# kekoveca/MPI-and-Open-MP

Hardware: AMD Instinct MI355X
Metric: Gcell-updates/sec at 1/2/4/8 MI355X + % of HBM roofline, bit-exact (higher is better)
Workload: dtype u32 (1 bit/cell)

## Files before the change

### include/life_mi355x.h

```cpp
#ifndef LIFE_MI355X_H
#define LIFE_MI355X_H

#include <stdint.h>

#ifdef __cplusplus
extern "C" {
#endif

#define LIFE_OK 0
#define LIFE_EINVAL (-1)
#define LIFE_EHIP (-2)
#define LIFE_ERCCL (-3)
#define LIFE_ENOMEM (-4)
#define LIFE_ESTATE (-5)
#define LIFE_EIO (-6)

#define LIFE_KERNEL_BYTE 0
#define LIFE_KERNEL_BIT 1

#define LIFE_XPORT_AUTO 0
#define LIFE_XPORT_RCCL 1
#define LIFE_XPORT_LOCAL 2

typedef struct life_dev life_dev;
// ... 81 lines not shown
int life_dev_checksum(life_dev *d, uint64_t *sum);


int life_dev_clear(life_dev *d);

int life_dev_set_cells(life_dev *d, const int64_t *xy, int64_t n, int alive);

int life_dev_upload_bits(life_dev *d, const uint8_t *packed);

int life_dev_gather_rect(life_dev *d, int64_t x0, int64_t y0, int64_t w, int64_t h, uint8_t *cells);

int life_dev_set_rect(life_dev *d, int64_t x0, int64_t y0, int64_t w, int64_t h, const uint8_t *cells);

int life_dev_gather_density(life_dev *d, int64_t fx, int64_t fy, uint32_t *counts);

int life_dev_sync(life_dev *d);
int life_dev_barrier(life_dev *d);
int life_device_count(void);
int life_dev_layout(life_dev *d, int local_shard, life_layout *out);
int life_dev_world(life_dev *d, int *world, int *dims0, int *dims1, int *nlocal, int *transport);
int life_dev_shard_info(life_dev *d, int local_shard, int *device, char pci_bus_id[64], int *rccl_nranks);

int life_dev_set_timing(life_dev *d, int on);

#define LIFE_OPT_SMALL_GRID 1
#define LIFE_OPT_OVERLAP 2
#define LIFE_OPT_BLOCK_GENS 5
#define LIFE_OPT_SMALL_WINDOW 4
#define LIFE_OPT_LOOPBACK 6
#define LIFE_OPT_FLOW 7
#define LIFE_OPT_FLOW_CHUNK 8
#define LIFE_OPT_DEEP_HALO 9
#define LIFE_OPT_PIPELINE 11
int life_dev_configure(life_dev *d, int option, int value);
#define LIFE_PATH_NONE 0
#define LIFE_PATH_ONEGEN 1
#define LIFE_PATH_TILES 2
#define LIFE_PATH_FLOW 3
#define LIFE_PATH_SMALL 5
int life_dev_last_path(life_dev *d);
int life_dev_kernel_stats(life_dev *d, double *avg_ms, int64_t *launches, double *bytes_per_launch);
int life_dev_kernel_work(life_dev *d, double *cell_updates_per_launch, double *valu_ops_per_launch);
int life_dev_phase_stats(life_dev *d, double *ring_ms, double *interior_ms, double *halo_ms, double *block_ms,
                         int64_t *blocks);
int life_dev_call_stats(life_dev *d, double *host_enqueue_ms, double *pass_enqueue_max_ms, int64_t *passes,
                        double *device_span_ms);

int life_tune(int kernel, int rows, int depth);

int life_tune_temporal(int kernel, int rows);

int life_measure_copy(int device, int64_t bytes, int reps, double *gbps);

void life_dev_destroy(life_dev *d);

#ifdef __cplusplus
}
#endif
#endif
```

### mpi-and-open-mp_amd/csrc/life_dev.hip

```cpp
#include <stdarg.h>

#include <chrono>
#include <thread>

#include "life_dev_internal.h"
#include "life_env.h"

using namespace life::rt;

thread_local std::string life::rt::g_err;

void life::rt::set_err(const char *fmt, ...) {
    char buf[512];
    va_list ap;
    va_start(ap, fmt);
    vsnprintf(buf, sizeof buf, fmt, ap);
    va_end(ap);
    g_err = buf;
}

static const int kEnvBlockGens = life::env::read(life::env::kBlockGens);
static const int kEnvFlow = life::env::read(life::env::kFlow);
static const bool kEnvDeepHalo = life::env::read(life::env::kDeepHalo) != 0;
static const int kEnvPipeline = [] {
    const int v = life::env::read(life::env::kPipeline);
    return v == 2 ? life::env::kPipeline.dflt : v;
}();
static int default_block_gens(int kernel) {
    return kEnvBlockGens ? kEnvBlockGens : (kernel == LIFE_KERNEL_BIT ? 12 : 32);
}

namespace {

int alloc_fill_byte() { return life::env::read(life::env::kPoison) ? 0xA5 : 0; }

int shard_alloc(Shard &s) {
    HIPCHK(hipSetDevice(s.device));
    HIPCHK(hipStreamCreateWithPriority(&s.stream, hipStreamNonBlocking, 0));
    HIPCHK(hipStreamCreateWithPriority(&s.stream2, hipStreamNonBlocking, 0));
    HIPCHK(hipStreamCreateWithPriority(&s.comm_stream, hipStreamNonBlocking, 0));
    const int fill = alloc_fill_byte();
    const int64_t slack = s.lay.generations_per_exchange > 1 ? life::kTemporalSlackRows : 0;
    const size_t bytes = (size_t)(s.lay.pitch * (s.lay.rows + slack));
    for (int i = 0; i < 2; i++) {
        HIPCHK(hipMalloc(&s.buf[i], bytes));
        HIPCHK(hipMemsetAsync(s.buf[i], fill, bytes, s.stream));
    }
    HIPCHK(hipEventCreateWithFlags(&s.ev_int, hipEventDisableTiming));
    HIPCHK(hipEventCreateWithFlags(&s.ev_halo, hipEventDisableTiming));
    HIPCHK(hipEventCreateWithFlags(&s.ev_sync, hipEventDisableTiming));
    HIPCHK(hipEventCreateWithFlags(&s.ev_entry, hipEventDisableTiming));
    for (hipEvent_t &e : s.ev_pipe) HIPCHK(hipEventCreateWithFlags(&e, hipEventDisableTiming));
    const size_t col_bytes = (size_t)life::column_stage_bytes(s.lay);
    HIPCHK(hipMalloc(&s.col_send, col_bytes));
    HIPCHK(hipMalloc(&s.col_recv, col_bytes));
    HIPCHK(hipMalloc(&s.d_count, 2 * sizeof(unsigned long long)));
    HIPCHK(hipMalloc(&s.sink, 1024));
    HIPCHK(hipMemsetAsync(s.col_send, fill, col_bytes, s.stream));
    HIPCHK(hipMemsetAsync(s.col_recv, fill, col_bytes, s.stream));
    HIPCHK(hipMemsetAsync(s.d_count, 0, 2 * sizeof(unsigned long long), s.stream));
// ... 37 lines not shown
        if (!s.comm) continue;
        HIPCHK(hipSetDevice(s.device));
        int64_t *h = reinterpret_cast<int64_t *>(s.h_count);
        h[0] = value;
        h[1] = -(int64_t)value;
        HIPCHK(hipMemcpyAsync(s.d_count, h, 2 * sizeof(int64_t), hipMemcpyHostToDevice, s.stream));
        NCCLCHK(ncclAllReduce(s.d_count, s.d_count, 2, ncclInt64, ncclMax, s.comm, s.stream));
        HIPCHK(hipMemcpyAsync(h, s.d_count, 2 * sizeof(int64_t), hipMemcpyDeviceToHost, s.stream));
        CHK(bounded_sync(s, what, -1));
        const int64_t hi = h[0], lo = -h[1];
        if (hi != lo) {
            set_err("%s is collective in rank mode: ranks passed %lld .. %lld", what, (long long)lo, (long long)hi);
            return LIFE_EINVAL;
        }
    }
    return LIFE_OK;
}

life_dev *new_dev(int64_t nx, int64_t ny, int dims0, int dims1, int world, int kernel) {
    int dims[2] = {dims0, dims1};
    if (dims0 <= 0 || dims1 <= 0) life_dims_create(world, dims);
    if (dims[0] * dims[1] != world) return nullptr;
    life_dev *d = new life_dev;
    d->nx = nx;
    d->ny = ny;
    d->dims[0] = dims[0];
    d->dims[1] = dims[1];
    d->world = world;
    d->kernel = kernel;
    d->block_gens = default_block_gens(kernel);
    d->deep = kEnvDeepHalo;
    d->flow = kEnvFlow;
    d->pipe = kEnvPipeline;
    return d;
}

int create_shards(life_dev *d, const std::vector<int> &ranks, const std::vector<int> &devices) {
    for (size_t i = 0; i < ranks.size(); i++) {
        d->shards.emplace_back();
        Shard &s = d->shards.back();
        s.rank = ranks[i];
        s.device = devices[i];
        const int rc = life_layout_query(d->nx, d->ny, d->dims[0], d->dims[1], s.rank, d->kernel, &s.lay);
        if (rc != LIFE_OK) {
            set_err("layout: nx=%lld ny=%lld dims=%dx%d rank %d kernel %d", (long long)d->nx,
                    (long long)d->ny, d->dims[0], d->dims[1], s.rank, d->kernel);
            return rc;
        }
    }
    for (Shard &s : d->shards) CHK(shard_alloc(s));
    return plan_halos(d);
}

void tail_prewarm(const life_dev *d) {
    for (size_t i = 0; i < d->shards.size(); ++i) {
        bool seen = false;
        for (size_t j = 0; j < i; ++j)
            seen |= d->shards[j].lay.w == d->shards[i].lay.w && d->shards[j].lay.h == d->shards[i].lay.h;
        if (!seen) life::prewarm_tail_plans(d->shards[i].lay, max_pass_gens(d), part(d, 1));
    }
}

int finish_create(life_dev *d, int rc, life_dev **out) {
    if (rc != LIFE_OK) {
        life_dev_destroy(d);
        return rc;
// ... 236 lines not shown
        if (value < 0 || value > 4) return LIFE_EINVAL;
        d->small_mode = value;
        return LIFE_OK;
    case LIFE_OPT_SMALL_WINDOW: {
        const int R = value >> 8, K = value & 255;
        if (value != 0 && (K < 1 || R < 1 || R > 8 || R == 7)) return LIFE_EINVAL;
        if (value != 0 && life::reg_win_plan(d->shards[0].lay, R, K).blocks == 0) {
            set_err("small-grid window R=%d K=%d does not fit this grid", R, K);
            return LIFE_EINVAL;
        }
        d->win_rows = R;
        d->win_halo = K;
        return LIFE_OK;
    }
    case LIFE_OPT_OVERLAP: d->overlap = value != 0; return LIFE_OK;
    case LIFE_OPT_BLOCK_GENS:
        if (value < 0 || value > 32) return LIFE_EINVAL;
        d->block_gens = value > 0 ? value : default_block_gens(d->kernel);
        tail_prewarm(d);
        return LIFE_OK;
    case LIFE_OPT_FLOW:
        if (value < 0 || value > 3) return LIFE_EINVAL;
        d->flow = value;
        return LIFE_OK;
    case LIFE_OPT_DEEP_HALO:
        if (value < 0 || value > 1) return LIFE_EINVAL;
        if (d->rank_mode && d->world > 1) CHK(agree_all_ranks(d, value, "LIFE_OPT_DEEP_HALO"));
        d->deep = value != 0;
        return LIFE_OK;
    case LIFE_OPT_PIPELINE:
        if (value < 0 || value == 2 || value > life::kPipeMaxRegions) return LIFE_EINVAL;
        d->pipe = value;
        return LIFE_OK;
    case LIFE_OPT_FLOW_CHUNK:
        if (value < 0) return LIFE_EINVAL;
        d->flow_chunk = value;
        return LIFE_OK;
    case LIFE_OPT_LOOPBACK: {
        if (value < 0 || value > 3) return LIFE_EINVAL;
        if (d->world != 1 || d->shards.size() != 1) {
            set_err("loopback needs a single-shard world (world %d, %zu local shards)", d->world, d->shards.size());
            return LIFE_EINVAL;
        }
        Shard &s = d->shards[0];
        if (value && (s.lay.h < s.lay.yapron || s.lay.w < s.lay.xapron)) {
            set_err("loopback: %lld x %lld cells < the %lld-column / %lld-row halo", (long long)s.lay.w,
                    (long long)s.lay.h, (long long)s.lay.xapron, (long long)s.lay.yapron);
            return LIFE_EINVAL;
        }
        if (value && d->transport == LIFE_XPORT_RCCL && !s.comm) {
            set_err("loopback over RCCL needs a communicator (life_dev_create_rank with a unique id, or "
                    "life_dev_create_ex with LIFE_XPORT_RCCL)");
            return LIFE_EINVAL;
        }
        d->loop = value == 0 ? 0 : value == 1 ? 3 : value == 2 ? 1 : 2;
        CHK(plan_halos(d));
        CHK(exchange(d, 0, false));
        tail_prewarm(d);
        return life_dev_sync(d);
    }
    default: return LIFE_EINVAL;
    }
}

int life_tune(int kernel, int rows, int depth) {
    if ((rows && rows != 16 && rows != 32 && rows != 64) ||
// ... 20 lines not shown
```

### mpi-and-open-mp_amd/csrc/life_dev_internal.h

```cpp
#pragma once
#include <rccl/rccl.h>
#include <stdio.h>
#include <string.h>

#include <algorithm>
#include <string>
#include <vector>

#include "life_host.h"
#include "life_io.h"
#include "life_kernels.h"
#include "life_mi355x.h"

#pragma GCC visibility push(hidden)

namespace life {
namespace rt {

extern thread_local std::string g_err;
void set_err(const char *fmt, ...);

#define HIPCHK(expr)                                                                          \
    do {                                                                                      \
        hipError_t e_ = (expr);                                                               \
// ... 63 lines not shown
    std::vector<int> slot;
    std::vector<LocalCopy> copies;
    std::vector<int> waits[2][2];
    std::vector<TimedLaunch> timers;
    size_t timers_used = 0;
    std::vector<PhaseEvents> phases;
    size_t phases_used = 0;
};

}
}

struct life_dev {
    int64_t nx = 0, ny = 0;
    int dims[2] = {1, 1};
    int world = 1;
    int kernel = LIFE_KERNEL_BYTE;
    int transport = LIFE_XPORT_LOCAL;
    bool rank_mode = false;
    bool timing = false;
    bool phase_events = true;
    bool launch_events = true;
    bool overlap = true;
    int block_gens = 0;
    int small_mode = 1;
    int win_rows = 0, win_halo = 0;
    int loop = 0;
    int last_path = LIFE_PATH_NONE;
    bool deep = true;
    int since = 0;
    int flow = 0;
    int64_t flow_chunk = 0;
    int pipe = 0;
    struct {
        int R = 0, m = 0;
        int64_t pass = 0;
        life::PipePlan plan;
    } pipe_call;
    life::rt::TimedLaunch *call_timer = nullptr;
    std::vector<life::rt::Shard> shards;
    double acc_ms = 0.0;
    int64_t acc_launches = 0;
    double acc_bytes = 0.0;
    double acc_updates = 0.0;
    double acc_valu = 0.0;
    double ph_ring = 0.0, ph_int = 0.0, ph_halo = 0.0, ph_block = 0.0;
    int64_t ph_blocks = 0;
    double call_host_ms = 0.0, call_pass_max_ms = 0.0;
    int64_t call_passes = 0;
    bool call_spans = false;
};

namespace life {
namespace rt {

inline bool part(const life_dev *d, int a) { return d->dims[a] > 1 || ((d->loop >> a) & 1); }
inline bool self_wrap_x(const life_dev *d) { return !(d->loop & 1) && life::self_wrap_x(d->shards[0].lay, d->dims[0]); }
inline life::Wrap wrap_of(const life_dev *d) { return life::Wrap{!part(d, 0) && !self_wrap_x(d), !part(d, 1)}; }
inline bool temporal(const life_dev *d) { return d->shards[0].lay.generations_per_exchange > 1; }
inline bool deep_halo(const life_dev *d) {
    return d->deep && d->kernel == LIFE_KERNEL_BIT && temporal(d) && (part(d, 0) || part(d, 1)) && !self_wrap_x(d);
}
inline int max_pass_gens(const life_dev *d) {
    return std::min(std::min(d->shards[0].lay.generations_per_exchange, 32), d->block_gens);
}
inline Shard *find_local(life_dev *d, int rank) {
// ... 32 lines not shown
```

### mpi-and-open-mp_amd/csrc/life_env.h

```cpp
#pragma once
#include <limits.h>
#include <stdlib.h>

#include "life_mi355x.h"

namespace life {
namespace env {

struct IntKnob { const char *name; int dflt, lo, hi; };
struct FlagKnob { const char *name; int dflt; };
struct RealKnob { const char *name; double dflt, lo, hi; };

inline int read(const IntKnob &k, int dflt) {
    const char *e = getenv(k.name);
    const int v = e ? atoi(e) : dflt;
    return v >= k.lo && v <= k.hi ? v : dflt;
}
inline int read(const IntKnob &k) { return read(k, k.dflt); }
inline int read(const FlagKnob &k) {
    const char *e = getenv(k.name);
    return e ? (atoi(e) != 0 ? 1 : 0) : k.dflt;
}
inline double read(const RealKnob &k) {
    const char *e = getenv(k.name);
    const double v = e ? atof(e) : k.dflt;
    return v > k.lo && v <= k.hi ? v : k.dflt;
}

constexpr IntKnob kStepRows{"LIFE_STEP_ROWS", 16, INT_MIN, INT_MAX};
constexpr IntKnob kStepDepth{"LIFE_STEP_DEPTH", 8, INT_MIN, INT_MAX};
constexpr FlagKnob kXcdOrderOnegen{"LIFE_XCD_ORDER_ONEGEN", -1};
constexpr IntKnob kTemporalRows{"LIFE_TEMPORAL_ROWS", 24, 16, 24};
constexpr IntKnob kTemporalRowsByte{"LIFE_TEMPORAL_ROWS_BYTE", 48, 32, 48};
constexpr FlagKnob kByteOneGhost{"LIFE_BYTE_ONE_GHOST", 1};
constexpr FlagKnob kBands{"LIFE_BANDS", 1};
constexpr FlagKnob kFlowBands{"LIFE_FLOW_BANDS", 1};
constexpr FlagKnob kXcdOrder{"LIFE_XCD_ORDER", 1};
constexpr FlagKnob kXcdOrderByte{"LIFE_XCD_ORDER_BYTE", 1};
constexpr IntKnob kTailSplit{"LIFE_TAIL_SPLIT", 2, 0, 2};
constexpr IntKnob kBlockGens{"LIFE_BLOCK_GENS", 0, 1, 32};
constexpr IntKnob kFlow{"LIFE_FLOW", 3, 0, 3};
constexpr FlagKnob kDeepHalo{"LIFE_DEEP_HALO", 1};
constexpr IntKnob kPipeline{"LIFE_PIPELINE", 1, 0, 16};
constexpr IntKnob kTimingMode{"LIFE_TIMING_MODE", 0, 0, 3};
constexpr FlagKnob kPoison{"LIFE_POISON", 0};
constexpr FlagKnob kInteriorTail{"LIFE_INTERIOR_TAIL", 0};
constexpr RealKnob kCommTimeoutS{"LIFE_COMM_TIMEOUT_S", 600.0, 0.0, 1e300};
constexpr IntKnob kTemporalDepth{"LIFE_TEMPORAL_DEPTH", LIFE_TEMPORAL_DEPTH, 1, 32};
constexpr IntKnob kTemporalDepthByte{"LIFE_TEMPORAL_DEPTH_BYTE", LIFE_TEMPORAL_DEPTH_BYTE, 1, 32};

}
}
```

### mpi-and-open-mp_amd/csrc/life_kernels.h

```cpp
#pragma once
#include <hip/hip_runtime.h>
#include <stdint.h>

#include "life_host.h"
#include "life_mi355x.h"

namespace life {

struct Region {
    int64_t u0, u1, r0, r1;
};

struct StepArgs {
    const uint8_t *in;
    uint8_t *out;
    uint8_t *sink;
    int64_t pitch, xoff, units, w, h, ya;
    int64_t u0, u1, r0, r1, nbx;
    int32_t wrapy;
    int32_t xcd;
};

struct Wrap {
    bool x, y;
// ... 8 lines not shown
StepTuning step_tuning(bool bit);
void set_step_tuning(int kernel, int rows, int depth);

constexpr int kMaxRegions = 4;
struct TileRegion {
    int64_t tx0, tx1, ty0, ty1;
};
struct TileGeom {
    int64_t lanes;
    int64_t cells;
    int64_t rows, ntx, nty;
    int gsh;
    int64_t bcol;
};
TileGeom tile_geom(const life_layout &L, int m);
int64_t region_items(const TileGeom &g, const TileRegion &r);
int tile_ghost(const life_layout &L, int m);
constexpr int64_t kTemporalSlackRows = 8 * 96;
bool flow_ok(const life_layout &L, int m);
int64_t flow_items_per_pass(const life_layout &L, int m, bool work_only = false);
int flow_slots(const life_layout &L);
int tile_slots(const life_layout &L);
hipError_t prewarm_tflow(const life_layout &L, int m, int flow, unsigned int *head, hipStream_t s);
hipError_t launch_tflow(const life_layout &L, const uint8_t *in, uint8_t *out, int m, int64_t passes,
                        unsigned int *head, unsigned int *done, Wrap wrap, int flow, hipStream_t s,
                        hipEvent_t ev0 = nullptr, hipEvent_t ev1 = nullptr);
struct Extend {
    int64_t y = 0;
    bool x = false;
};
hipError_t launch_tstep(const life_layout &L, const uint8_t *in, uint8_t *out, const TileRegion *r, int nreg,
                        int m, Wrap wrap, hipStream_t s,
                        double *valu_lane_ops = nullptr, hipEvent_t ev0 = nullptr, hipEvent_t ev1 = nullptr,
                        Extend ext = Extend{}, int64_t concurrent = 0);
void prewarm_tail_plans(const life_layout &L, int mmax, bool ext_y);
life_layout extended_layout(const life_layout &L, const Extend &ext);
int temporal_rows(bool bit);
int tile_waves(bool bit);
double tstep_valu_per_tile_lane(int m, bool byte);
void set_temporal_rows(int kernel, int nr);

constexpr int64_t kSmallMaxLds = 160 * 1024;
int64_t small_lds_bytes(const life_layout &L);
hipError_t launch_small(const life_layout &L, const uint8_t *in, uint8_t *out, int64_t gens, hipStream_t s);
int reg_small_rows(const life_layout &L);
hipError_t launch_reg_small(const life_layout &L, const uint8_t *in, uint8_t *out, int64_t gens,
                            hipStream_t s);
struct RegWinPlan {
    int R, K, ns, own, blocks;
};
RegWinPlan reg_win_plan(const life_layout &L, int R, int K);
hipError_t launch_reg_win(const life_layout &L, const RegWinPlan &p, const uint8_t *in, uint8_t *out, int gens,
                          hipStream_t s, bool nat_in, bool nat_out);

}
```

### mpi-and-open-mp_amd/csrc/life_kernels.hip

```cpp
#include "life_kernels.h"
#include "life_bitops.h"
#include "life_diag.h"
#include "life_env.h"

#include <hip/hip_ext.h>

#include <algorithm>
#include <stdint.h>

namespace life {
namespace {

constexpr int kBlock = 256;

__device__ __forceinline__ uint32_t from_left(uint32_t old, uint32_t v) {
    return (uint32_t)__builtin_amdgcn_update_dpp((int)old, (int)v, 0x138, 0xf, 0xf, false);
}
__device__ __forceinline__ uint32_t from_right(uint32_t old, uint32_t v) {
    return (uint32_t)__builtin_amdgcn_update_dpp((int)old, (int)v, 0x130, 0xf, 0xf, false);
}

struct ByteEnc {
    static constexpr int64_t kCellsPerUnit = 16;
    static constexpr uint32_t kCell0 = 0xFFu;
    static __device__ __forceinline__ int64_t dword_of(int64_t x) { return x >> 2; }
    static __device__ __forceinline__ uint32_t pos_in_dword(int64_t x) { return 8u * (uint32_t)(x & 3); }
    static __device__ __forceinline__ uint32_t top_shift(int64_t x) { return 24u - pos_in_dword(x); }
    struct H {
        uint32_t v[4];
    };
    static __device__ __forceinline__ H hsum(uint4 d, uint32_t l, uint32_t r) {
        H h;
        h.v[0] = d.x + __builtin_amdgcn_alignbyte(d.x, l, 3) + __builtin_amdgcn_alignbyte(d.y, d.x, 1);
        h.v[1] = d.y + __builtin_amdgcn_alignbyte(d.y, d.x, 3) + __builtin_amdgcn_alignbyte(d.z, d.y, 1);
        h.v[2] = d.z + __builtin_amdgcn_alignbyte(d.z, d.y, 3) + __builtin_amdgcn_alignbyte(d.w, d.z, 1);
        h.v[3] = d.w + __builtin_amdgcn_alignbyte(d.w, d.z, 3) + __builtin_amdgcn_alignbyte(r, d.w, 1);
        return h;
    }
    static __device__ __forceinline__ uint32_t rule1(uint32_t n9, uint32_t c) {
        const uint32_t m = (n9 - c) | c;
        const uint32_t t = m ^ 0x03030303u;
// ... 159 lines not shown
                const uint32_t m = E::kCell0 << E::pos_in_dword(q);
                c.pshift = E::pos_in_dword(q);
                c.pmask.x = comp == 0 ? m : 0u;
                c.pmask.y = comp == 1 ? m : 0u;
                c.pmask.z = comp == 2 ? m : 0u;
                c.pmask.w = comp == 3 ? m : 0u;
            }
        }
    }
    const bool st = u < a.u1;
    uint8_t *dst = st ? a.out + (ys + a.ya) * a.pitch + a.xoff + 16 * u : a.sink + 16 * lane;
    const int64_t spitch = st ? a.pitch : 0;
    const int64_t n = a.r1 - ys < R ? a.r1 - ys : R;
    if (n == R)
        strip_full<E, R, D, WRAPX>(c, ys, dst, spitch);
    else
        strip_tail<E, WRAPX>(c, ys, (int)n, dst, spitch);
}


constexpr int kStackWaves = 8;
struct TArgs {
    const uint8_t *in;
    uint8_t *out;
    int64_t pitch, xoff, W, h, ya;
    int64_t tx0[kMaxRegions], tx1[kMaxRegions], ty0[kMaxRegions], ty1[kMaxRegions], first[kMaxRegions + 1];
    int32_t nreg, m;
    int32_t gsh;
    int64_t bcol;
    int64_t tail_first, tail_y, tail_yend, tail_ntx, tail_tx0;
    int32_t tail_band;
    int64_t xcd_n;
    int32_t xext;
};

template <int NW>
using Xch = uint32_t[2][NW][4][64];
template <int NW>
using XchP = uint32_t[2][NW + 2][8][64];
template <int NW>
struct XchB {
    XchP<NW> s;
};

#ifndef LIFE_FLOW_BP_AHEAD
#define LIFE_FLOW_BP_AHEAD 1
#endif
#ifndef LIFE_FAST_WRAP
#define LIFE_FAST_WRAP 1
#endif

template <int R, bool WRAPX, bool WRAPY, int FLOW, int NW, bool BAND = false>
__device__ __forceinline__ void tile_body_bit(const TArgs &a, const uint8_t *in, uint8_t *out, int64_t tx,
                                              int64_t ty, XchB<NW> &xb, int gsh = 6, int nb = 1,
                                              int64_t ybase = 0, int64_t yend = -1) {
    XchP<NW> &xch = xb.s;
    static_assert(R >= 3, "window");
    const int K = a.m;
    const int T = NW * R - 2 * K;
    const int lane = threadIdx.x & 63;
    const int laddr = ((lane - 1) & 63) << 2, raddr = ((lane + 1) & 63) << 2;
    const int wi = __builtin_amdgcn_readfirstlane(threadIdx.x >> 6);
    const int gl = BAND ? lane >> gsh : 0;
    const int pin = BAND ? lane & ((1 << gsh) - 1) : lane;
    const int64_t j = tx * 62 + pin - 1;
    int64_t jl;
    if (WRAPX) {
        if (LIFE_FAST_WRAP && a.W >= 64) {
            jl = j < 0 ? j + a.W : (j >= a.W ? j - a.W : j);
        } else {
            jl = j % a.W;
            if (jl < 0) jl += a.W;
        }
    } else {
        jl = j > a.W ? a.W : j;
    }
    const uint32_t voff = (uint32_t)(a.xoff + 8 * jl);
    const int64_t y0 = ybase + ty * T - K + (int64_t)wi * R;
    const uint8_t *row0 = in + a.ya * a.pitch;
    uint32_t ve[R], vo[R];
    {
        int64_t y = y0 + (BAND ? (int64_t)(gl < nb ? gl : nb - 1) * T : 0);
        if (WRAPY) {
            if (LIFE_FAST_WRAP && a.h > 65 * (int64_t)(NW * R)) {
                y = y < 0 ? y + a.h : (y >= a.h ? y - a.h : y);
            } else {
                y %= a.h;
                if (y < 0) y += a.h;
            }
        }
        const uint8_t *p = row0 + y * a.pitch;
#pragma unroll
        for (int r = 0; r < R; ++r) {
            uint64_t q;
            if (FLOW)
                q = __hip_atomic_load(reinterpret_cast<uint64_t *>(const_cast<uint8_t *>(p) + voff),
                                      __ATOMIC_RELAXED, __HIP_MEMORY_SCOPE_AGENT);
            else
                q = *reinterpret_cast<const uint64_t *>(p + voff);
            ve[r] = (uint32_t)q;
            vo[r] = (uint32_t)(q >> 32);
            ++y;
            if (WRAPY && y == a.h) {
                y = 0;
                p = row0;
            } else {
                p += a.pitch;
            }
        }
    }
    auto hsum = [&](uint32_t e, uint32_t o, uint32_t &e0, uint32_t &e1, uint32_t &o0, uint32_t &o1) {
        BitEnc::pair_sums(e, o, bperm(laddr, o), bperm(raddr, e), e0, e1, o0, o1);
    };
    if (wi == 0 || wi == NW - 1)
        for (int q = 0; q < 16; ++q) xch[q >> 3][wi == 0 ? 0 : NW + 1][q & 7][lane] = 0u;
    for (int g = 0; g < a.m; ++g) {
        const int par = g & 1;
        uint32_t pe0, pe1, po0, po1, ce0, ce1, co0, co1;
        {
            uint32_t be0, be1, bo0, bo1;
            hsum(ve[R - 1], vo[R - 1], be0, be1, bo0, bo1);
            xch[par][wi + 1][4][lane] = be0;
            xch[par][wi + 1][5][lane] = be1;
            xch[par][wi + 1][6][lane] = bo0;
            xch[par][wi + 1][7][lane] = bo1;
        }
        hsum(ve[0], vo[0], pe0, pe1, po0, po1);
        xch[par][wi + 1][0][lane] = pe0;
        xch[par][wi + 1][1][lane] = pe1;
        xch[par][wi + 1][2][lane] = po0;
        xch[par][wi + 1][3][lane] = po1;
        __syncthreads();
        hsum(ve[1], vo[1], ce0, ce1, co0, co1);
        {
            const uint32_t ae0 = xch[par][wi][4][lane], ae1 = xch[par][wi][5][lane];
            const uint32_t ao0 = xch[par][wi][6][lane], ao1 = xch[par][wi][7][lane];
            ve[0] = BitEnc::rule1(ae0, ae1, pe0, pe1, ce0, ce1, ve[0]);
            vo[0] = BitEnc::rule1(ao0, ao1, po0, po1, co0, co1, vo[0]);
        }
        constexpr int BAH = FLOW ? LIFE_FLOW_BP_AHEAD : 0;
        uint32_t bl[BAH > 0 ? BAH : 1], br[BAH > 0 ? BAH : 1];
#pragma unroll
        for (int k = 0; k < BAH; ++k)
            if (2 + k < R - 1) {
                bl[k] = bperm(laddr, vo[2 + k]);
                br[k] = bperm(raddr, ve[2 + k]);
            }
#pragma unroll
        for (int r = 1; r < R - 1; ++r) {
// ... 5 lines not shown
                no1 = xch[par][wi + 1][7][lane];
            } else if (BAH > 0) {
                const uint32_t l = bl[0], rr = br[0];
#pragma unroll
                for (int k = 0; k + 1 < BAH; ++k) {
                    bl[k] = bl[k + 1];
                    br[k] = br[k + 1];
                }
                if (r + 1 + BAH < R - 1) {
                    bl[BAH - 1] = bperm(laddr, vo[r + 1 + BAH]);
                    br[BAH - 1] = bperm(raddr, ve[r + 1 + BAH]);
                }
                __builtin_amdgcn_sched_barrier(0);
                BitEnc::pair_sums(ve[r + 1], vo[r + 1], l, rr, ne0, ne1, no0, no1);
            } else {
                hsum(ve[r + 1], vo[r + 1], ne0, ne1, no0, no1);
            }
            ve[r] = BitEnc::rule1(pe0, pe1, ce0, ce1, ne0, ne1, ve[r]);
            vo[r] = BitEnc::rule1(po0, po1, co0, co1, no0, no1, vo[r]);
            pe0 = ce0;
            pe1 = ce1;
            po0 = co0;
            po1 = co1;
            ce0 = ne0;
            ce1 = ne1;
            co0 = no0;
            co1 = no1;
        }
        {
            const uint32_t de0 = xch[par][wi + 2][0][lane], de1 = xch[par][wi + 2][1][lane];
            const uint32_t do0 = xch[par][wi + 2][2][lane], do1 = xch[par][wi + 2][3][lane];
            ve[R - 1] = BitEnc::rule1(pe0, pe1, ce0, ce1, de0, de1, ve[R - 1]);
            vo[R - 1] = BitEnc::rule1(po0, po1, co0, co1, do0, do1, vo[R - 1]);
        }
    }
    const int r0 = min(max(K - wi * R, 0), R), r1 = min(max(NW * R - K - wi * R, 0), R);
    int lane2 = (int)(threadIdx.x & 63);
    asm volatile("" : "+v"(lane2));
    const int gl2 = BAND ? lane2 >> gsh : 0;
    const int pin2 = BAND ? lane2 & ((1 << gsh) - 1) : lane2;
    const int64_t j2 = tx * 62 + pin2 - 1;
    const bool st = (BAND ? (pin2 >= 1 && pin2 <= (1 << gsh) - 2 && j2 < a.W && gl2 < nb)
                          : (lane2 >= 1 && lane2 <= 62 && j2 < a.W)) ||
                    (!WRAPX && a.xext && (!BAND || gl2 < nb) && (j2 == -1 || j2 == a.W));
    const int64_t yb = y0 + (BAND ? (int64_t)(gl2 < nb ? gl2 : 0) * T : 0);
    const int64_t ylim = yend >= 0 ? yend : a.h;
    uint8_t *q = out + (a.ya + yb + r0) * a.pitch + voff;
#pragma unroll
    for (int r = 0; r < R; ++r) {
        if (r < r0 || r >= r1) continue;
        if (st && yb + r < ylim) {
            const uint64_t v = (uint64_t)ve[r] | ((uint64_t)vo[r] << 32);
            if (FLOW == 1)
                __hip_atomic_store(reinterpret_cast<uint64_t *>(q), v, __ATOMIC_RELAXED, __HIP_MEMORY_SCOPE_AGENT);
            else
                *reinterpret_cast<uint64_t *>(q) = v;
        }
        q += a.pitch;
    }
}

#ifndef LIFE_BYTE_WPE
#define LIFE_BYTE_WPE 4
#endif
#ifndef LIFE_BYTE_LOAD_CHUNK
#define LIFE_BYTE_LOAD_CHUNK 0
// ... 139 lines not shown
    const int64_t ntxs = a.tail_ntx - (band ? 1 : 0), nfull = ntxs * rows;
    if (i < nfull) {
        tile_body_bit<RS, WRAPX, WRAPY, 0, NW>(a, a.in, a.out, a.tail_tx0 + i % ntxs, i / ntxs, xch, 6, 1, y0,
                                              yend);
    } else {
        const int64_t B = 64 >> a.gsh, ty = (i - nfull) * B;
        const int nb = (int)(rows - ty < B ? rows - ty : B);
        tile_body_bit<RS, WRAPX, WRAPY, 0, NW, true>(a, a.in, a.out, a.bcol, ty, xch, a.gsh, nb, y0, yend);
    }
}

template <int R, bool WRAPX, bool WRAPY, int NW>
__global__ __launch_bounds__(64 * NW, bit_wpe(NW, R)) void tstep_bit_kernel(TArgs a) {
    __shared__ XchB<NW> xch;
    wg_trace(0);
    int64_t wg = blockIdx.x;
    if (wg < a.xcd_n) {
        const int64_t n = a.xcd_n, x = wg & 7, k = wg >> 3, per = n >> 3, rem = n & 7;
        wg = (x < rem ? x * (per + 1) : rem * (per + 1) + (x - rem) * per) + k;
    }
    if (a.tail_ntx > 0 && wg >= a.tail_first) {
        tail_item<R / 2, WRAPX, WRAPY, NW>(a, wg - a.tail_first, xch);
        wg_trace(1);
        return;
    }
    const int64_t nwg = a.first[a.nreg];
    if (wg >= nwg) return;
    int k = 0;
    while (k + 1 < a.nreg && wg >= a.first[k + 1]) ++k;
    const int64_t wr = wg - a.first[k];
    const bool bands = a.gsh < 6 && a.tx1[k] == a.bcol + 1;
    const int64_t ntx = a.tx1[k] - a.tx0[k] - (bands ? 1 : 0);
    const int64_t nfull = ntx * (a.ty1[k] - a.ty0[k]);
    if (wr < nfull) {
        const int64_t tx = a.tx0[k] + wr % ntx, ty = a.ty0[k] + wr / ntx;
        tile_body_bit<R, WRAPX, WRAPY, 0, NW>(a, a.in, a.out, tx, ty, xch);
    } else {
        const int64_t B = 64 >> a.gsh, ty = a.ty0[k] + (wr - nfull) * B;
        const int nb = (int)(a.ty1[k] - ty < B ? a.ty1[k] - ty : B);
        tile_body_bit<R, WRAPX, WRAPY, 0, NW, true>(a, a.in, a.out, a.bcol, ty, xch, a.gsh, nb);
    }
    wg_trace(1);
}

template <int R, int GK, bool WRAPX, bool WRAPY, int NW>
__global__ __launch_bounds__(64 * NW, LIFE_BYTE_WPE) void tstep_byte_kernel(TArgs a) {
    __shared__ Xch<NW> xch;
    wg_trace(0);
    int64_t wg = blockIdx.x;
    if (wg < a.xcd_n) {
        const int64_t n = a.xcd_n, x = wg & 7, k = wg >> 3, per = n >> 3, rem = n & 7;
        wg = (x < rem ? x * (per + 1) : rem * (per + 1) + (x - rem) * per) + k;
    }
    const int64_t nwg = a.first[a.nreg];
    if (wg >= nwg) return;
    int k = 0;
    while (k + 1 < a.nreg && wg >= a.first[k + 1]) ++k;
    const int64_t wr = wg - a.first[k];
    const int64_t ntx = a.tx1[k] - a.tx0[k];
    const int64_t tx = a.tx0[k] + wr % ntx, ty = a.ty0[k] + wr / ntx;
    tile_body_byte<R, GK, WRAPX, WRAPY, NW>(a, a.in, a.out, tx, ty, xch);
}

struct FArgs {
    TArgs t;
    int64_t ntx, nty, items;
    int64_t per_pass, ngroups, B;
    unsigned int *head;
    unsigned int *done;
};

template <int R, bool WRAPX, bool WRAPY, int FLOW, int NW, bool BAND = false>
__global__ __launch_bounds__(64 * NW, bit_wpe(NW, R)) void tflow_kernel(FArgs f) {
// ... 564 lines not shown
life_layout extended_layout(const life_layout &L, const Extend &ext) {
    life_layout V = L;
    V.h += 2 * ext.y;
    V.yapron -= ext.y;
    V.rows = V.h + 2 * V.yapron;
    return V;
}

static int64_t region_bands(const TileGeom &g, int64_t tx1) { return g.gsh < 6 && tx1 == g.bcol + 1 ? 64 >> g.gsh : 1; }

static TailPlan tail_plan_for(const life_layout &L, const TileGeom &g, int m, int64_t tx0, int64_t tx1, int64_t ty0,
                              int64_t ty1, int64_t pre) {
    const int64_t T2 = (int64_t)tile_waves(true) * (temporal_rows(true) / 2) - 2 * (int64_t)tile_ghost(L, m);
    const int64_t yend = std::min(ty1 * g.rows, L.h);
    return tail_plan(tx1 - tx0, region_bands(g, tx1), ty0, ty1, yend, g.rows, T2, tstep_bit_slots(),
                     tail_split_mode(), kTailC, pre);
}

void prewarm_tail_plans(const life_layout &L, int mmax, bool ext_y) {
    if (!is_bit(L) || L.generations_per_exchange < 2 || tail_split_mode() == 0) return;
    const int K = L.generations_per_exchange;
    for (int m = 1; m <= std::min(mmax, K); ++m)
        for (int e = 0; e <= (ext_y ? K - m : 0); ++e) {
            Extend x;
            x.y = e;
            const life_layout V = extended_layout(L, x);
            const TileGeom g = tile_geom(V, m);
            if (g.rows >= 1) (void)tail_plan_for(V, g, m, 0, g.ntx, 0, g.nty, 0);
        }
}

hipError_t launch_tstep(const life_layout &Lin, const uint8_t *in, uint8_t *out, const TileRegion *r, int nreg,
                        int m, Wrap wrap, hipStream_t s, double *valu_lane_ops, hipEvent_t ev0, hipEvent_t ev1,
                        Extend ext, int64_t concurrent) {
    const int K = Lin.generations_per_exchange;
    const bool bit = is_bit(Lin);
    if (nreg < 0 || nreg > kMaxRegions || m > K || m > 32 || K < 2 || Lin.yapron != K || ext.y < 0 ||
        ((ext.y > 0 || ext.x) && (!bit || ext.y + m > K || (ext.y > 0 && wrap.y) || (ext.x && wrap.x))) ||
        tile_waves(bit) * temporal_rows(bit) - 2 * tile_ghost(Lin, m) < 1 || (!bit && K != 16 && K != 32))
        return hipErrorInvalidValue;
    const life_layout L = extended_layout(Lin, ext);
    const TileGeom g = tile_geom(L, m);
    TArgs a;
    a.in = in;
    a.out = out;
    a.pitch = L.pitch;
    a.xoff = L.xoff;
    a.W = (L.w + g.cells - 1) / g.cells;
    a.h = L.h;
    a.ya = L.yapron;
    a.m = m;
    a.xext = ext.x ? 1 : 0;
    a.nreg = 0;
    a.first[0] = 0;
    a.gsh = (int32_t)g.gsh;
    a.bcol = g.bcol;
    for (int k = 0; k < nreg; k++) {
        if (r[k].tx1 <= r[k].tx0 || r[k].ty1 <= r[k].ty0) continue;
        const int n = a.nreg++;
        a.tx0[n] = r[k].tx0;
        a.tx1[n] = r[k].tx1;
        a.ty0[n] = r[k].ty0;
        a.ty1[n] = r[k].ty1;
        a.first[n + 1] = a.first[n] + region_items(g, r[k]);
    }
    if (a.nreg == 0 || m <= 0) return hipSuccess;
    int64_t items = a.first[a.nreg];
    a.tail_first = a.tail_y = a.tail_yend = a.tail_ntx = a.tail_tx0 = 0;
    a.tail_band = 0;
    const int64_t T2 = (int64_t)tile_waves(bit) * (temporal_rows(bit) / 2) - 2 * (int64_t)tile_ghost(L, m);
    if (bit && T2 >= 1 && a.nreg == 1 && tail_split_mode() > 0 && concurrent >= 0) {
        const int64_t tx0 = a.tx0[0], tx1 = a.tx1[0], ty0 = a.ty0[0], ty1 = a.ty1[0];
        const int64_t yend = std::min(ty1 * g.rows, L.h), B = region_bands(g, tx1);
        const TailPlan p = tail_plan_for(L, g, m, tx0, tx1, ty0, ty1, concurrent);
        if (p.F < ty1 && p.F >= ty0) {
            a.ty1[0] = p.F;
            a.first[1] = region_items(g, TileRegion{tx0, tx1, ty0, p.F});
            a.tail_first = a.first[1];
            a.tail_y = p.F * g.rows;
            a.tail_yend = yend;
            a.tail_ntx = tx1 - tx0;
            a.tail_tx0 = tx0;
            a.tail_band = B > 1 ? 1 : 0;
            items = a.tail_first + tail_row_items(tx1 - tx0, B, p.n2);
        }
// ... 226 lines not shown
```

### mpi-and-open-mp_amd/csrc/life_step.hip

```cpp
#include <chrono>
#include <utility>

#include "life_dev_internal.h"
#include "life_env.h"

using namespace life::rt;

constexpr double kFlowAutoRounds = 5.0;
constexpr int64_t kFlowMinPasses = 4;

namespace {

int launch_region(life_dev *d, Shard &s, const life::Region &r, bool timed, hipStream_t st) {
    Bracket b;
    CHK(bracket_begin(d, s, timed, 1, kExtNever, false, st, &b));
    HIPCHK(life::launch_step(s.lay, s.buf[s.cur], s.buf[s.cur ^ 1], s.sink, r, wrap_of(d), st));
    CHK(bracket_end(b, st));
    if (b.t) {
        const bool bit = s.lay.kernel == LIFE_KERNEL_BIT;
        const int64_t cpu = bit ? 128 : 16;
        const int64_t xa = r.u0 * cpu, xb = r.u1 * cpu < s.lay.w ? r.u1 * cpu : s.lay.w;
        book(d, bit, (double)(xb - xa) * (double)(r.r1 - r.r0), 1.0, 1.0, 0.0);
    }
    return LIFE_OK;
}

int launch_tiles(life_dev *d, Shard &s, const life::TileRegion *r, int nreg, int m, bool timed, hipStream_t st,
                 life::Extend xt = life::Extend{}, int64_t concurrent = 0) {
    Bracket b;
    CHK(bracket_begin(d, s, timed, 1, kExtModeExt | kExtModeCall, false, st, &b));
    double valu = 0.0;
    HIPCHK(life::launch_tstep(s.lay, s.buf[s.cur], s.buf[s.cur ^ 1], r, nreg, m, wrap_of(d), st, &valu, b.ext_a,
                              b.ext_b, xt, concurrent));
    CHK(bracket_end(b, st));
    if (b.t) {
        const life::TileGeom g = life::tile_geom(life::extended_layout(s.lay, xt), m);
        double cells = 0.0;
        for (int k = 0; k < nreg; k++) {
            const int64_t xa = r[k].tx0 * g.lanes * g.cells, xb = std::min(r[k].tx1 * g.lanes * g.cells, s.lay.w);
            const int64_t ya = std::max(r[k].ty0 * g.rows - xt.y, (int64_t)0),
                          yb = std::min(r[k].ty1 * g.rows - xt.y, s.lay.h);
            if (xb > xa && yb > ya) cells += (double)(xb - xa) * (double)(yb - ya);
        }
        book(d, s.lay.kernel == LIFE_KERNEL_BIT, cells, (double)m, 1.0, valu);
    }
    return LIFE_OK;
}


constexpr int kPipeAutoRegions = 4;
constexpr double kPipeAutoRounds = 1.0;
constexpr int64_t kPipeAutoPasses = 4;

int64_t tile_bands(const life::TileGeom &g) { return g.gsh < 6 ? 64 >> g.gsh : 1; }

int fence_stream2(Shard &s) {
    HIPCHK(hipEventRecord(s.ev_entry, s.stream));
    HIPCHK(hipStreamWaitEvent(s.stream2, s.ev_entry, 0));
    return LIFE_OK;
}
int join_stream2(Shard &s) {
    HIPCHK(hipEventRecord(s.ev_int, s.stream2));
    HIPCHK(hipStreamWaitEvent(s.stream, s.ev_int, 0));
    return LIFE_OK;
}

int pipelined_pass(life_dev *d, Shard &s, int m) {
    auto &pc = d->pipe_call;
    const life::TileGeom g = life::tile_geom(s.lay, m);
    if (pc.m != m) {
        if (pc.m != 0) {
            CHK(join_stream2(s));
            CHK(fence_stream2(s));
        }
        pc.plan = life::pipe_plan(g.nty, tile_bands(g), pc.R, 2);
        pc.m = m;
        pc.pass = 0;
    }
    const life::PipePlan &P = pc.plan;
    if (P.R == 0) {
        const life::TileRegion all{0, g.ntx, 0, g.nty};
        return launch_tiles(d, s, &all, 1, m, true, s.stream);
    }
    Bracket b;
    CHK(bracket_begin(d, s, true, 1, kExtNever, false, s.stream, &b));
    hipStream_t st[2] = {s.stream, s.stream2};
    double valu = 0.0;
    for (int j = 0; j < P.R; j++) {
        const int64_t i = pc.pass * P.R + j;
        const int r = (int)((pc.pass + j) % P.R);
        hipStream_t q = st[i % 2];
        if (pc.pass > 0)
            for (int w = 0; w < P.nwait[j]; w++)
                HIPCHK(hipStreamWaitEvent(q, s.ev_pipe[(i - P.wait[j][w]) % kPipeRing], 0));
        const life::TileRegion reg{0, g.ntx, P.ty[r], P.ty[r + 1]};
        double v = 0.0;
        HIPCHK(life::launch_tstep(s.lay, s.buf[s.cur], s.buf[s.cur ^ 1], &reg, 1, m, wrap_of(d), q, &v, nullptr,
                                  nullptr, life::Extend{}, -1));
        valu += v;
        if (P.record[j]) HIPCHK(hipEventRecord(s.ev_pipe[i % kPipeRing], q));
    }
    CHK(bracket_end(b, s.stream));
    if (b.t) book(d, s.lay.kernel == LIFE_KERNEL_BIT, (double)s.lay.w * (double)s.lay.h, (double)m, 1.0, valu);
    pc.pass++;
    return LIFE_OK;
}

bool interior_tail() { static const bool v = life::env::read(life::env::kInteriorTail) != 0; return v; }


int phase_begin(life_dev *d, Shard &s, PhaseEvents **pe) {
    *pe = nullptr;
    if (!d->timing || !d->phase_events) return LIFE_OK;
    int rc;
    *pe = phase_slot(s, &rc);
    if (!*pe) return rc;
    HIPCHK(hipEventRecord((*pe)->ring0, s.stream));
    return LIFE_OK;
}
int phase_ring(Shard &s, PhaseEvents *pe) {
    if (pe) {
        HIPCHK(hipEventRecord(pe->ring1, s.stream));
        HIPCHK(hipEventRecord(pe->halo0, s.stream));
    }
    return LIFE_OK;
}
int phase_end(life_dev *d, const std::vector<PhaseEvents *> &pe, const std::vector<char> &halo_side) {
    for (size_t si = 0; si < d->shards.size(); ++si) {
        Shard &s = d->shards[si];
        HIPCHK(hipSetDevice(s.device));
        if (pe[si]) HIPCHK(hipEventRecord(pe[si]->halo1, s.stream));
// ... 422 lines not shown
```

### mpi-and-open-mp_amd/life_mi355x/__init__.py

```python
from __future__ import annotations

import ctypes
import importlib.abc
import os
import sys

import numpy as np

from .cfg import (bits_bytes, density_bytes, load_bits, load_bits_packed, load_cfg, load_cfg_cells,
                  load_density, save_vtk, vtk_bytes, vtk_header)

HERE = os.path.dirname(os.path.abspath(__file__))
LIB_PATH = os.environ.get("LIFE_MI355X_LIB") or os.path.join(HERE, "liblife_mi355x.so")

KERNEL_BYTE = 0
KERNEL_BIT = 1
KERNELS = {"byte": KERNEL_BYTE, "bit": KERNEL_BIT}
XPORT_AUTO, XPORT_RCCL, XPORT_LOCAL = 0, 1, 2
HALO_SEND, HALO_RECV, HALO_FILL = 0, 1, 2
HALO_COLUMN, HALO_ROW, HALO_CORNER = 0, 1, 2
OPT_SMALL_GRID, OPT_OVERLAP, OPT_SMALL_WINDOW, OPT_BLOCK_GENS, OPT_LOOPBACK, OPT_FLOW = 1, 2, 4, 5, 6, 7
OPT_FLOW_CHUNK = 8
OPT_DEEP_HALO = 9
OPT_PIPELINE = 11
TEMPORAL_DEPTH = {"bit": 32, "byte": 32}
BLOCK_GENS = {"bit": 12, "byte": 32}
TEMPORAL_ROWS = {"bit": 24, "byte": 48}
TILE_WAVES = {"bit": 8, "byte": 8}
TEMPORAL_XAPRON = {"bit": 64, "byte": 32}

ABI_SYMBOLS = (
    "life_decomposition", "life_dims_create", "life_dims_choose", "life_halo_plan", "life_layout_query",
    "life_strerror", "life_last_error", "life_dev_create", "life_dev_create_ex",
    "life_get_unique_id", "life_dev_create_rank", "life_dev_upload", "life_dev_fill_random",
    "life_dev_step", "life_dev_gather", "life_dev_live_count", "life_dev_sync",
    "life_dev_layout", "life_dev_world", "life_dev_set_timing", "life_dev_kernel_stats",
    "life_tune", "life_tune_temporal", "life_dev_configure", "life_dev_kernel_work", "life_dev_checksum",
    "life_dev_gather_vtk", "life_dev_gather_bits", "life_dev_destroy", "life_measure_copy", "life_dev_phase_stats",
    "life_dev_barrier", "life_device_count", "life_dev_last_path", "life_dev_call_stats",
    "life_dev_strerror", "life_dev_shard_info",
    "life_dev_clear", "life_dev_set_cells", "life_dev_gather_rect", "life_dev_gather_density",
    "life_dev_upload_bits", "life_dev_set_rect",
)
PATHS = {0: "none", 1: "onegen", 2: "tiles", 3: "flow", 5: "small"}


class LifeError(RuntimeError):
    def __init__(self, rc: int, what: str):
        lib = _lib()
        detail = lib.life_last_error().decode(errors="replace")
        super().__init__(f"{what}: {lib.life_strerror(rc).decode()} ({rc}){': ' + detail if detail else ''}")
        self.rc = rc


class HaloOp(ctypes.Structure):
    _fields_ = [("phase", ctypes.c_int32), ("kind", ctypes.c_int32), ("peer", ctypes.c_int32),
                ("what", ctypes.c_int32), ("index", ctypes.c_int64), ("first", ctypes.c_int64),
# ... 369 lines not shown
```

Baseline: 124,500.

## Trim ghost-row recomputation in edge waves of temporal bit tiles

Adds a ghost-trim mode, on by default (LIFE_GHOST_TRIM=2), for the bit-packed temporally blocked tile kernel. The first and last waves of a tile stop running full-height generations after a few steps and instead update a shrinking window of rows, in chunks of trim depth. This skips redundant apron work whose results are later discarded. In exchange it adds register swaps to flip the top wave, extra template instantiations and a separate generation loop. There is some risk of divergence between waves and higher register pressure.

```diff
diff --git a/include/life_mi355x.h b/include/life_mi355x.h
--- a/include/life_mi355x.h
+++ b/include/life_mi355x.h
@@ -137,6 +137,7 @@
 #define LIFE_OPT_FLOW_CHUNK 8
 #define LIFE_OPT_DEEP_HALO 9
 #define LIFE_OPT_PIPELINE 11
+#define LIFE_OPT_GHOST_TRIM 12
 int life_dev_configure(life_dev *d, int option, int value);
 #define LIFE_PATH_NONE 0
 #define LIFE_PATH_ONEGEN 1
diff --git a/mpi-and-open-mp_amd/csrc/life_dev.hip b/mpi-and-open-mp_amd/csrc/life_dev.hip
--- a/mpi-and-open-mp_amd/csrc/life_dev.hip
+++ b/mpi-and-open-mp_amd/csrc/life_dev.hip
@@ -26,6 +26,7 @@
     const int v = life::env::read(life::env::kPipeline);
     return v == 2 ? life::env::kPipeline.dflt : v;
 }();
+static const int kEnvGhostTrim = life::env::read(life::env::kGhostTrim);
 static int default_block_gens(int kernel) {
     return kEnvBlockGens ? kEnvBlockGens : (kernel == LIFE_KERNEL_BIT ? 12 : 32);
 }
@@ -129,6 +130,7 @@
     d->deep = kEnvDeepHalo;
     d->flow = kEnvFlow;
     d->pipe = kEnvPipeline;
+    d->trim = kEnvGhostTrim;
     return d;
 }
 
@@ -431,6 +433,10 @@
         if (value < 0 || value == 2 || value > life::kPipeMaxRegions) return LIFE_EINVAL;
         d->pipe = value;
         return LIFE_OK;
+    case LIFE_OPT_GHOST_TRIM:
+        if (value < 0 || value > 4) return LIFE_EINVAL;
+        d->trim = value;
+        return LIFE_OK;
     case LIFE_OPT_FLOW_CHUNK:
         if (value < 0) return LIFE_EINVAL;
         d->flow_chunk = value;
diff --git a/mpi-and-open-mp_amd/csrc/life_dev_internal.h b/mpi-and-open-mp_amd/csrc/life_dev_internal.h
--- a/mpi-and-open-mp_amd/csrc/life_dev_internal.h
+++ b/mpi-and-open-mp_amd/csrc/life_dev_internal.h
@@ -119,6 +119,7 @@
     int flow = 0;
     int64_t flow_chunk = 0;
     int pipe = 0;
+    int trim = 0;
     struct {
         int R = 0, m = 0;
         int64_t pass = 0;
diff --git a/mpi-and-open-mp_amd/csrc/life_env.h b/mpi-and-open-mp_amd/csrc/life_env.h
--- a/mpi-and-open-mp_amd/csrc/life_env.h
+++ b/mpi-and-open-mp_amd/csrc/life_env.h
@@ -42,6 +42,7 @@
 constexpr IntKnob kFlow{"LIFE_FLOW", 3, 0, 3};
 constexpr FlagKnob kDeepHalo{"LIFE_DEEP_HALO", 1};
 constexpr IntKnob kPipeline{"LIFE_PIPELINE", 1, 0, 16};
+constexpr IntKnob kGhostTrim{"LIFE_GHOST_TRIM", 2, 0, 4};
 constexpr IntKnob kTimingMode{"LIFE_TIMING_MODE", 0, 0, 3};
 constexpr FlagKnob kPoison{"LIFE_POISON", 0};
 constexpr FlagKnob kInteriorTail{"LIFE_INTERIOR_TAIL", 0};
diff --git a/mpi-and-open-mp_amd/csrc/life_kernels.h b/mpi-and-open-mp_amd/csrc/life_kernels.h
--- a/mpi-and-open-mp_amd/csrc/life_kernels.h
+++ b/mpi-and-open-mp_amd/csrc/life_kernels.h
@@ -64,7 +64,7 @@
 hipError_t launch_tstep(const life_layout &L, const uint8_t *in, uint8_t *out, const TileRegion *r, int nreg,
                         int m, Wrap wrap, hipStream_t s,
                         double *valu_lane_ops = nullptr, hipEvent_t ev0 = nullptr, hipEvent_t ev1 = nullptr,
-                        Extend ext = Extend{}, int64_t concurrent = 0);
+                        Extend ext = Extend{}, int64_t concurrent = 0, int trim = 0);
 void prewarm_tail_plans(const life_layout &L, int mmax, bool ext_y);
 life_layout extended_layout(const life_layout &L, const Extend &ext);
 int temporal_rows(bool bit);
diff --git a/mpi-and-open-mp_amd/csrc/life_kernels.hip b/mpi-and-open-mp_amd/csrc/life_kernels.hip
--- a/mpi-and-open-mp_amd/csrc/life_kernels.hip
+++ b/mpi-and-open-mp_amd/csrc/life_kernels.hip
@@ -7,6 +7,7 @@
 
 #include <algorithm>
 #include <stdint.h>
+#include <type_traits>
 
 namespace life {
 namespace {
@@ -232,7 +233,31 @@
     int32_t tail_band;
     int64_t xcd_n;
     int32_t xext;
+    int32_t trim;
 };
+
+#ifndef LIFE_TRIM_STEP
+#define LIFE_TRIM_STEP 3
+#endif
+#ifndef LIFE_TRIM_BUILD
+#define LIFE_TRIM_BUILD 1
+#endif
+#ifndef LIFE_TRIM_ROT
+#define LIFE_TRIM_ROT 0
+#endif
+constexpr int kTrimStep = LIFE_TRIM_STEP, kTrimMaxS = 12;
+constexpr int trim_rows(int g, int R) {
+    const int smax = kTrimMaxS < R - 3 ? kTrimMaxS : R - 3;
+    const int s = 1 + g / kTrimStep * kTrimStep;
+    return s == 1 ? 0 : s <= smax ? s : 1 + (smax - 1) / kTrimStep * kTrimStep;
+}
+template <int S, int R, class F>
+__device__ __forceinline__ void trim_chunks(F &f, int m) {
+    constexpr bool last = trim_rows(S - 1 + kTrimStep, R) == S;
+    const int g0 = S - 1, g1 = last ? m : min(m, g0 + kTrimStep);
+    if (g0 < m) f(std::integral_constant<int, S>{}, g0, g1);
+    if constexpr (!last) trim_chunks<S + kTrimStep, R>(f, m);
+}
 
 template <int NW>
 using Xch = uint32_t[2][NW][4][64];
@@ -250,17 +275,19 @@
 #define LIFE_FAST_WRAP 1
 #endif
 
-template <int R, bool WRAPX, bool WRAPY, int FLOW, int NW, bool BAND = false>
+template <int R, bool WRAPX, bool WRAPY, int FLOW, int NW, bool BAND = false, bool TRIM = false>
 __device__ __forceinline__ void tile_body_bit(const TArgs &a, const uint8_t *in, uint8_t *out, int64_t tx,
                                               int64_t ty, XchB<NW> &xb, int gsh = 6, int nb = 1,
-                                              int64_t ybase = 0, int64_t yend = -1) {
+                                              int64_t ybase = 0, int64_t yend = -1, int rot = 0, bool trim = false) {
     XchP<NW> &xch = xb.s;
     static_assert(R >= 3, "window");
+    static_assert(!TRIM || (FLOW == 0 && R >= 6 && (NW & (NW - 1)) == 0), "ghost trim: per-launch tiles");
     const int K = a.m;
     const int T = NW * R - 2 * K;
     const int lane = threadIdx.x & 63;
     const int laddr = ((lane - 1) & 63) << 2, raddr = ((lane + 1) & 63) << 2;
-    const int wi = __builtin_amdgcn_readfirstlane(threadIdx.x >> 6);
+    const int wi = __builtin_amdgcn_readfirstlane(TRIM && LIFE_TRIM_ROT ? (int)((threadIdx.x >> 6) + rot) & (NW - 1)
+                                                                        : (int)(threadIdx.x >> 6));
     const int gl = BAND ? lane >> gsh : 0;
     const int pin = BAND ? lane & ((1 << gsh) - 1) : lane;
     const int64_t j = tx * 62 + pin - 1;
@@ -312,9 +339,11 @@
     auto hsum = [&](uint32_t e, uint32_t o, uint32_t &e0, uint32_t &e1, uint32_t &o0, uint32_t &o1) {
         BitEnc::pair_sums(e, o, bperm(laddr, o), bperm(raddr, e), e0, e1, o0, o1);
     };
+    const bool trimmed = TRIM && trim && (wi == 0 || wi == NW - 1);
+    const int gfull = trimmed ? min(a.m, kTrimStep) : a.m;
     if (wi == 0 || wi == NW - 1)
         for (int q = 0; q < 16; ++q) xch[q >> 3][wi == 0 ? 0 : NW + 1][q & 7][lane] = 0u;
-    for (int g = 0; g < a.m; ++g) {
+    for (int g = 0; g < gfull; ++g) {
         const int par = g & 1;
         uint32_t pe0, pe1, po0, po1, ce0, ce1, co0, co1;
         {
@@ -386,6 +415,61 @@
             const uint32_t do0 = xch[par][wi + 2][2][lane], do1 = xch[par][wi + 2][3][lane];
             ve[R - 1] = BitEnc::rule1(pe0, pe1, ce0, ce1, de0, de1, ve[R - 1]);
             vo[R - 1] = BitEnc::rule1(po0, po1, co0, co1, do0, do1, vo[R - 1]);
+        }
+    }
+    if constexpr (TRIM) {
+        if (trimmed) {
+            const bool top = wi == 0;
+            auto flip = [&]() {
+#pragma unroll
+                for (int r = 0; r < R / 2; ++r) {
+                    asm volatile("v_swap_b32 %0, %1" : "+v"(ve[r]), "+v"(ve[R - 1 - r]));
+                    asm volatile("v_swap_b32 %0, %1" : "+v"(vo[r]), "+v"(vo[R - 1 - r]));
+                }
+            };
+            if (top) flip();
+            const int pw = wi + 1, pk = top ? 4 : 0;
+            const int nw = top ? 2 : NW - 1, nk = top ? 0 : 4;
+            auto gens = [&](auto s_, int g0, int g1) {
+                constexpr int S = decltype(s_)::value;
+                static_assert(S >= 2 && S <= R - 3, "trim depth");
+#pragma unroll
+                for (int r = R - S + 1; r < R; ++r) ve[r] = vo[r] = 0u;
+                for (int g = g0; g < g1; ++g) {
+                    const int par = g & 1;
+                    uint32_t pe0, pe1, po0, po1, ce0, ce1, co0, co1;
+                    hsum(ve[0], vo[0], pe0, pe1, po0, po1);
+                    xch[par][pw][pk + 0][lane] = pe0;
+                    xch[par][pw][pk + 1][lane] = pe1;
+                    xch[par][pw][pk + 2][lane] = po0;
+                    xch[par][pw][pk + 3][lane] = po1;
+                    __syncthreads();
+                    hsum(ve[1], vo[1], ce0, ce1, co0, co1);
+                    {
+                        const uint32_t ae0 = xch[par][nw][nk + 0][lane], ae1 = xch[par][nw][nk + 1][lane];
+                        const uint32_t ao0 = xch[par][nw][nk + 2][lane], ao1 = xch[par][nw][nk + 3][lane];
+                        ve[0] = BitEnc::rule1(ae0, ae1, pe0, pe1, ce0, ce1, ve[0]);
+                        vo[0] = BitEnc::rule1(ao0, ao1, po0, po1, co0, co1, vo[0]);
+                    }
+#pragma unroll
+                    for (int r = 1; r < R - S; ++r) {
+                        uint32_t ne0, ne1, no0, no1;
+                        hsum(ve[r + 1], vo[r + 1], ne0, ne1, no0, no1);
+                        ve[r] = BitEnc::rule1(pe0, pe1, ce0, ce1, ne0, ne1, ve[r]);
+                        vo[r] = BitEnc::rule1(po0, po1, co0, co1, no0, no1, vo[r]);
+                        pe0 = ce0;
+                        pe1 = ce1;
+                        po0 = co0;
+                        po1 = co1;
+                        ce0 = ne0;
+                        ce1 = ne1;
+                        co0 = no0;
+                        co1 = no1;
+                    }
+                }
+            };
+            trim_chunks<1 + kTrimStep, R>(gens, a.m);
+            if (top) flip();
         }
     }
     const int r0 = min(max(K - wi * R, 0), R), r1 = min(max(NW * R - K - wi * R, 0), R);
@@ -591,13 +675,17 @@
     const bool bands = a.gsh < 6 && a.tx1[k] == a.bcol + 1;
     const int64_t ntx = a.tx1[k] - a.tx0[k] - (bands ? 1 : 0);
     const int64_t nfull = ntx * (a.ty1[k] - a.ty0[k]);
+    const bool trim = a.trim == 1 || a.trim == 2 || a.trim == 4;
+    const int rot = !LIFE_TRIM_ROT ? 0 : a.trim == 1 || a.trim == 3 ? (int)(wg & (NW - 1) & 3) : a.trim == 4 ? (int)(wg & 1) * 2 : 0;
     if (wr < nfull) {
         const int64_t tx = a.tx0[k] + wr % ntx, ty = a.ty0[k] + wr / ntx;
-        tile_body_bit<R, WRAPX, WRAPY, 0, NW>(a, a.in, a.out, tx, ty, xch);
+        tile_body_bit<R, WRAPX, WRAPY, 0, NW, false, LIFE_TRIM_BUILD != 0>(a, a.in, a.out, tx, ty, xch, 6, 1, 0, -1, rot,
+                                                                           trim);
     } else {
         const int64_t B = 64 >> a.gsh, ty = a.ty0[k] + (wr - nfull) * B;
         const int nb = (int)(a.ty1[k] - ty < B ? a.ty1[k] - ty : B);
-        tile_body_bit<R, WRAPX, WRAPY, 0, NW, true>(a, a.in, a.out, a.bcol, ty, xch, a.gsh, nb);
+        tile_body_bit<R, WRAPX, WRAPY, 0, NW, true, LIFE_TRIM_BUILD != 0>(a, a.in, a.out, a.bcol, ty, xch, a.gsh, nb, 0, -1,
+                                                                          rot, trim);
     }
     wg_trace(1);
 }
@@ -1228,7 +1316,7 @@
 
 hipError_t launch_tstep(const life_layout &Lin, const uint8_t *in, uint8_t *out, const TileRegion *r, int nreg,
                         int m, Wrap wrap, hipStream_t s, double *valu_lane_ops, hipEvent_t ev0, hipEvent_t ev1,
-                        Extend ext, int64_t concurrent) {
+                        Extend ext, int64_t concurrent, int trim) {
     const int K = Lin.generations_per_exchange;
     const bool bit = is_bit(Lin);
     if (nreg < 0 || nreg > kMaxRegions || m > K || m > 32 || K < 2 || Lin.yapron != K || ext.y < 0 ||
@@ -1247,6 +1335,7 @@
     a.ya = L.yapron;
     a.m = m;
     a.xext = ext.x ? 1 : 0;
+    a.trim = bit && trim >= 0 && trim <= 4 ? trim : 0;
     a.nreg = 0;
     a.first[0] = 0;
     a.gsh = (int32_t)g.gsh;
diff --git a/mpi-and-open-mp_amd/csrc/life_step.hip b/mpi-and-open-mp_amd/csrc/life_step.hip
--- a/mpi-and-open-mp_amd/csrc/life_step.hip
+++ b/mpi-and-open-mp_amd/csrc/life_step.hip
@@ -31,7 +31,7 @@
     CHK(bracket_begin(d, s, timed, 1, kExtModeExt | kExtModeCall, false, st, &b));
     double valu = 0.0;
     HIPCHK(life::launch_tstep(s.lay, s.buf[s.cur], s.buf[s.cur ^ 1], r, nreg, m, wrap_of(d), st, &valu, b.ext_a,
-                              b.ext_b, xt, concurrent));
+                              b.ext_b, xt, concurrent, d->trim));
     CHK(bracket_end(b, st));
     if (b.t) {
         const life::TileGeom g = life::tile_geom(life::extended_layout(s.lay, xt), m);
@@ -96,7 +96,7 @@
         const life::TileRegion reg{0, g.ntx, P.ty[r], P.ty[r + 1]};
         double v = 0.0;
         HIPCHK(life::launch_tstep(s.lay, s.buf[s.cur], s.buf[s.cur ^ 1], &reg, 1, m, wrap_of(d), q, &v, nullptr,
-                                  nullptr, life::Extend{}, -1));
+                                  nullptr, life::Extend{}, -1, d->trim));
         valu += v;
         if (P.record[j]) HIPCHK(hipEventRecord(s.ev_pipe[i % kPipeRing], q));
     }
diff --git a/mpi-and-open-mp_amd/life_mi355x/__init__.py b/mpi-and-open-mp_amd/life_mi355x/__init__.py
--- a/mpi-and-open-mp_amd/life_mi355x/__init__.py
+++ b/mpi-and-open-mp_amd/life_mi355x/__init__.py
@@ -23,6 +23,7 @@
 OPT_FLOW_CHUNK = 8
 OPT_DEEP_HALO = 9
 OPT_PIPELINE = 11
+OPT_GHOST_TRIM = 12
 TEMPORAL_DEPTH = {"bit": 32, "byte": 32}
 BLOCK_GENS = {"bit": 12, "byte": 32}
 TEMPORAL_ROWS = {"bit": 24, "byte": 48}
diff --git a/profiles/ghost_trim/ab.py b/profiles/ghost_trim/ab.py
--- /dev/null
+++ b/profiles/ghost_trim/ab.py
@@ -0,0 +1,58 @@
+import json
+import os
+import subprocess
+import sys
+import time
+
+ROOT = os.path.dirname(os.path.dirname(os.path.dirname(os.path.abspath(__file__))))
+P = {"LIFE_MI355X_LIB": os.environ.get("LIFE_AB_PARENT_LIB", "")}
+
+
+def T(v):
+    return {"LIFE_GHOST_TRIM": str(v)}
+
+
+def arms(name):
+    if name == "arms":
+        return [("parent", P, []), ("trim_rot", T(1), []), ("off", T(0), []), ("trim", T(2), []), ("rot", T(3), []),
+                ("trim_rot02", T(4), [])] * 4
+    a = {"final": [],
+         "driver": ["--steps", "20", "--warmup", "5"],
+         "half": ["--shape", "16384x32768"],
+         "byte": ["--kernel", "byte"]}.get(name)
+    if a is None:
+        raise SystemExit(f"unknown set {name}")
+    one = [("parent", P, a), ("default", {}, a), ("off", T(0), a)]
+    return one + one[::-1] + one[1:] + one[:1] + one[::-1]
+
+
+def main():
+    name, path = sys.argv[1], sys.argv[2]
+    if not os.path.exists(P["LIFE_MI355X_LIB"]):
+        raise SystemExit("LIFE_AB_PARENT_LIB: the parent commit's liblife_mi355x.so")
+    with open(path, "a") as out:
+        for label, env, args in arms(name):
+            t0 = time.time()
+            try:
+                r = subprocess.run([sys.executable, os.path.join(ROOT, "bench.py"), *args],
+                                   env=dict(os.environ, **env), capture_output=True, text=True, timeout=150, cwd=ROOT)
+            except subprocess.TimeoutExpired:
+                print(f"{label}: time limit, stopping", flush=True)
+                return 1
+            lines = [ln for ln in r.stdout.splitlines() if ln.startswith("{")]
+            if r.returncode != 0 or len(lines) != 1:
+                print(f"{label}: rc {r.returncode}\n{r.stdout[-1500:]}\n{r.stderr[-1500:]}", flush=True)
+                return 1
+            j = json.loads(lines[0])
+            issued = j.get("roofline", {}).get("issued", {})
+            rec = dict(set=name, arm=label, value=j["value"], live=j.get("config", {}).get("live_cells_end"),
+                       ms_per_step=j.get("ms_per_step"), issued_frac=issued.get("frac"),
+                       ops_per_launch=issued.get("ops_per_launch"), call=j.get("call"), wall_s=round(time.time() - t0, 1))
+            out.write(json.dumps(rec) + "\n")
+            out.flush()
+            print(f"{label:12s} {j['value']:10.3f} Gcell/s  span {j.get('call', {}).get('device_span_ms')} ms", flush=True)
+    return 0
+
+
+if __name__ == "__main__":
+    sys.exit(main())
```

New measurement: 124,900, median of 6. No clear change (+0.3%).
